# Samleo8/RadarSLAMPy

Hardware: AMD Instinct MI355X
Metric: radar scan-pairs/sec (400x3768 polar) (higher is better)
Workload: dtype u8/f32/f64

## Files before the change

radarslampy_amd/csrc/engine.hip:

```cpp
#include "roam_internal.h"
#include "retrack.h"
#include "kabsch_body.inc"
#include <algorithm>
#include <new>

#define KS ROAM_MAX_FEATURES
#define CART_CENTER 1012.0
#define M_PER_PX 0.0864
#define N_RETRACK 60
#define ROT_THR 0.2
#define TRANS_THR_SQ 4.0
#define ERR_THR 10.0f
#define TWO_PI 6.283185307179586476925286766559

#define RES_RING 8
enum { ST_PEAKS = 0, ST_WARP, ST_PYR, ST_KLT, ST_GRAPH, ST_CLIQUE, ST_KABSCH, ST_LM, ST_GLUE, ST_RETRACK, ST_COUNT };
static const char *kStageNames[ST_COUNT] = {"ingest_peaks", "warp_quantise", "pyramid", "klt", "consistency_graph",
                                            "max_clique", "kabsch", "mds_lm", "glue", "retrack"};

struct Engine {
    roam_engine_cfg cfg;
    int B = 0, W = 0, stage_cap = 0;
    PyrDesc pd;
    size_t rec_bytes = 0;
// ... 39 lines not shown
    hipEvent_t ev_pool = nullptr;
    bool pool_dirty = false;
    RtArgs rt;
    bool rt_on = false;
    int rt_mode = 1;
    uint8_t *kfb = nullptr;
    uint8_t *rmap = nullptr;
    int rmap_cap = 0;
    int64_t rmap_n = 0;
    int64_t rmap_n_bcast = 0;
    std::vector<int32_t> rmap_root;
    uint8_t *kfx_send = nullptr, *kfx_recv = nullptr;
    size_t kfx_rec = 0;
    int kfx_peaks = 0;
    int kfx_world = 0;
    int64_t *rmap_n_dev = nullptr;
    int32_t *rmap_root_dev = nullptr;
    int64_t kfx_calls = 0;
    bool kfx_ready = false;
    hipStream_t st_comm = nullptr;
    hipEvent_t ev_kfx[3] = {};
    int kfx_last = -1;
    hipEvent_t ev[ST_COUNT + 1] = {};
    bool stage_ev_forced = false;
    bool stage_ev = true;
    hipEvent_t ev_join = nullptr, ev_pk0 = nullptr, ev_pk1 = nullptr;
    hipEvent_t ev_klt[4] = {}, ev_g4[4] = {};
    hipEvent_t ev_warp = nullptr;
    hipEvent_t ev_idx = nullptr, ev_peaks = nullptr;
    hipEvent_t tr_ev[64][6] = {};
    hipEvent_t rt_ev[64][3 * RT_TRACE_CHUNKS] = {};
    bool rt_ev_ok[64] = {};
    hipEvent_t ev_emit = nullptr;
    RtSide det_side = {};
    int det_chunk() const { return (det_side.chunk > 0 && retrack_sided(rt, B, &det_side)) ? det_side.chunk : rt.slots; }
    int64_t rt_image_px = 0;
    bool tr_ev_ok[64] = {};
    int64_t stage_ev_step = -1;
    bool tr_ok = false;
    unsigned long long *pyr_dark = nullptr;
    static constexpr bool warp_dark_zero = true;
    bool ev_ok = false, stepped = false, uploads_pending = false;
    uint64_t up_seq = 0, up_waited = 0;
    std::vector<uint64_t> slot_seq;
    hipEvent_t ev_up_ring[16] = {};
    std::vector<int> lane_k;
// ... 76 lines not shown
            good_new[2 * o] = klt_next[2 * i]; good_new[2 * o + 1] = klt_next[2 * i + 1];
            good_idx[o] = k;
            pos++;
        }
    }
    if (t == 0) good_n[b] = total;
}

__global__ void fill_mask_kernel(uint8_t *mask, const int32_t *good_n, int32_t *cq_n, int32_t *cq_flags)
{
    const int b = blockIdx.x;
    for (int k = threadIdx.x; k < KS; k += blockDim.x) mask[(int64_t)b * KS + k] = 1;
    if (threadIdx.x == 0) { cq_n[b] = good_n[b]; cq_flags[b] = 1; }
}

__global__ __launch_bounds__(256) void g2_inliers_kernel(const float *__restrict__ good_old, const float *__restrict__ good_new,
                                                         const int32_t *__restrict__ good_idx, const int32_t *__restrict__ good_n,
                                                         const uint8_t *__restrict__ mask, const double *__restrict__ kf_pose,
                                                         const double *__restrict__ kf_und, double *__restrict__ kf_und_tmp,
                                                         double *__restrict__ kab_src, double *__restrict__ kab_tgt,
                                                         double *__restrict__ p_w, double *__restrict__ p_jt,
                                                         float *__restrict__ feat, int32_t *__restrict__ in_n,
                                                         double *__restrict__ kab_out, const double *__restrict__ pose,
                                                         double *__restrict__ T_wj0, double *__restrict__ T_init)
{
    __shared__ int sh[8];
    __shared__ double red[8];
    const int b = blockIdx.x, t = threadIdx.x;
    const int G = good_n[b];
    const int items = (KS + 255) / 256;
    const int lo = t * items, hi = min(lo + items, G);
    int c = 0;
    for (int g = lo; g < hi; g++) c += mask[(int64_t)b * KS + g] ? 1 : 0;
    int total;
    int pos = blk_excl_scan(c, sh, &total);
    const double kx = kf_pose[3 * b], ky = kf_pose[3 * b + 1], kth = kf_pose[3 * b + 2];
    const double ck = cos(kth), sk = sin(kth);
    for (int g = lo; g < hi; g++) {
        const int64_t i = (int64_t)b * KS + g;
        if (!mask[i]) continue;
        const int64_t o = (int64_t)b * KS + pos;
        const float ox = good_old[2 * i], oy = good_old[2 * i + 1];
        const float nx = good_new[2 * i], ny = good_new[2 * i + 1];
        kab_src[2 * o] = (double)ox; kab_src[2 * o + 1] = (double)oy;
        kab_tgt[2 * o] = (double)nx; kab_tgt[2 * o + 1] = (double)ny;
        const int64_t ki = (int64_t)b * KS + good_idx[i];
        const double ux = kf_und[2 * ki], uy = kf_und[2 * ki + 1];
        kf_und_tmp[2 * o] = ux; kf_und_tmp[2 * o + 1] = uy;
        p_w[2 * o] = ck * ux - sk * uy + kx;
        p_w[2 * o + 1] = sk * ux + ck * uy + ky;
        p_jt[2 * o] = ((double)nx - CART_CENTER) * M_PER_PX;
        p_jt[2 * o + 1] = ((double)ny - CART_CENTER) * M_PER_PX;
        pos++;
    }
    __syncthreads();
    pos -= c;
    for (int g = lo; g < hi; g++) {
        const int64_t i = (int64_t)b * KS + g;
        if (!mask[i]) continue;
        const int64_t o = (int64_t)b * KS + pos;
        feat[2 * o] = good_new[2 * i]; feat[2 * o + 1] = good_new[2 * i + 1];
        pos++;
    }
    if (t == 0) in_n[b] = total;
    __threadfence_block();
    __syncthreads();
    double *ko = kab_out + 6 * (int64_t)b;
    kabsch_body(kab_src + (int64_t)b * KS * 2, kab_tgt + (int64_t)b * KS * 2, total, red, ko);
    if (T_wj0 && t == 0) {
        const double x = pose[3 * b], y = pose[3 * b + 1], th = pose[3 * b + 2];
        const double c = cos(th), s = sin(th);
        double *T0 = T_wj0 + 9 * (int64_t)b, *Ti = T_init + 9 * (int64_t)b;
        T0[0] = c; T0[1] = -s; T0[2] = x; T0[3] = s; T0[4] = c; T0[5] = y; T0[6] = 0; T0[7] = 0; T0[8] = 1;
        const double hx = ko[4] * M_PER_PX, hy = ko[5] * M_PER_PX;
        Ti[0] = c * ko[0] - s * ko[2]; Ti[1] = c * ko[1] - s * ko[3]; Ti[2] = c * hx - s * hy + x;
        Ti[3] = s * ko[0] + c * ko[2]; Ti[4] = s * ko[1] + c * ko[3]; Ti[5] = s * hx + c * hy + y;
        Ti[6] = 0; Ti[7] = 0; Ti[8] = 1;
    }
}


#define MAP_SLOT (8 + 2 * KS)
__device__ __forceinline__ void map_freeze(double *__restrict__ map_store, int32_t *__restrict__ map_n, int map_cap, int b,
                                           const double *__restrict__ kfp, const double *__restrict__ kfv, int n,
                                           int scan, const double *__restrict__ locals)
{
    const int slot = map_n[b];
    if (slot >= map_cap) return;
    double *d = map_store + ((size_t)b * map_cap + slot) * MAP_SLOT;
    for (int j = threadIdx.x; j < 2 * n; j += blockDim.x) d[8 + j] = locals[j];
    if (threadIdx.x == 0) {
        d[0] = kfp[0]; d[1] = kfp[1]; d[2] = kfp[2];
        d[3] = kfv[0]; d[4] = kfv[1]; d[5] = kfv[2];
        d[6] = (double)n; d[7] = (double)scan;
    }
}

__global__ __launch_bounds__(256) void map_freeze_kernel(double *__restrict__ map_store, int32_t *__restrict__ map_n, int map_cap,
                                                         int b, const double *__restrict__ kf_pose,
                                                         const double *__restrict__ kf_vel, const int32_t *__restrict__ feat_n,
                                                         const int32_t *__restrict__ kf_scan, const double *__restrict__ kf_und,
                                                         const int32_t *__restrict__ kf_live, const int32_t *__restrict__ kf_fresh)
{
    if (!kf_live[b] || kf_fresh[b]) return;
    const int slot = map_n[b];
    map_freeze(map_store, map_n, map_cap, b, kf_pose + 3 * b, kf_vel + 3 * b, feat_n[b], kf_scan[b], kf_und + (size_t)b * KS * 2);
    __syncthreads();
    if (threadIdx.x == 0 && slot < map_cap) map_n[b] = slot + 1;
}

__global__ __launch_bounds__(256) void g4_update_kernel(roam_engine_cfg cfg, const double *__restrict__ lm_out,
                                                        const int32_t *__restrict__ lm_nfev, const int32_t *__restrict__ lm_info,
                                                        const double *__restrict__ kab_out, double *__restrict__ pose,
                                                        double *__restrict__ vel, double *__restrict__ kf_pose,
                                                        double *__restrict__ kf_und, const double *__restrict__ kf_und_tmp,
                                                        const double *__restrict__ p_jt, const int32_t *__restrict__ in_n,
                                                        const int32_t *__restrict__ good_n, int32_t *__restrict__ feat_n,
                                                        const int32_t *__restrict__ peaks_n, const int32_t *__restrict__ cq_flags,
                                                        roam_lane_result *__restrict__ res, const int32_t *__restrict__ scan_idx,
                                                        double *__restrict__ kf_vel, int32_t *__restrict__ kf_scan,
                                                        int32_t *__restrict__ kf_fresh, const int32_t *__restrict__ kf_live,
                                                        double *__restrict__ map_store, int32_t *__restrict__ map_n, int map_cap,
                                                        int collect, int32_t *__restrict__ rt_lane, int32_t *__restrict__ rt_scan,
                                                        int32_t *__restrict__ rt_n)
{
    __shared__ double np_[3], nv_[3];
    __shared__ int newkf;
    const int b = blockIdx.x, t = threadIdx.x;
    const int n = in_n[b];
    if (t == 0) {
        double px = pose[3 * b], py = pose[3 * b + 1], pth = pose[3 * b + 2];
        double v0 = 0, v1 = 0, v2 = 0;
        const double *k = kab_out + 6 * (int64_t)b;
        if (n >= 2) {
            if (cfg.motion_distortion) {
                const double *s = lm_out + 6 * (int64_t)b;
                v0 = s[0]; v1 = s[1]; v2 = s[2]; px = s[3]; py = s[4]; pth = s[5];
            } else {
                const double dx = k[4] * M_PER_PX, dy = k[5] * M_PER_PX, dth = atan2(k[2], k[0]);
                const double c = cos(pth), s = sin(pth);
                px += dx * c - dy * s; py += dx * s + dy * c; pth += dth;
            }
        }
        np_[0] = px; np_[1] = py; np_[2] = pth; nv_[0] = v0; nv_[1] = v1; nv_[2] = v2;
        const int retrack = n <= N_RETRACK;
        const double dth = fabs(kf_pose[3 * b + 2] - pth);
        const double ddx = kf_pose[3 * b] - px, ddy = kf_pose[3 * b + 1] - py;
        const int good = (dth >= cfg.keyframe_rot_rad) || (ddx * ddx + ddy * ddy >= cfg.keyframe_trans_m * cfg.keyframe_trans_m);
        newkf = retrack || good;
        roam_lane_result *r = res + b;
        r->pose[0] = px; r->pose[1] = py; r->pose[2] = pth;
        r->velocity[0] = v0; r->velocity[1] = v1; r->velocity[2] = v2;
        r->kabsch_R[0] = k[0]; r->kabsch_R[1] = k[1]; r->kabsch_R[2] = k[2]; r->kabsch_R[3] = k[3];
        r->kabsch_h[0] = k[4] * M_PER_PX; r->kabsch_h[1] = k[5] * M_PER_PX;
        r->n_tracked = feat_n[b]; r->n_good = good_n[b]; r->n_inliers = n; r->n_peaks = peaks_n[b];
        r->lm_nfev = (n >= 2 && cfg.motion_distortion) ? lm_nfev[b] : 0;
        r->lm_info = (n >= 2 && cfg.motion_distortion) ? lm_info[b] : 0;
        __hip_atomic_store(&r->flags, (cq_flags[b] & 1) | (newkf ? 2 : 0) | (retrack ? 4 : 0), __ATOMIC_RELAXED, __HIP_MEMORY_SCOPE_AGENT);
        r->n_after_retrack = 0;
    }
    __syncthreads();
    const double v0 = nv_[0], v1 = nv_[1], v2 = nv_[2];
    const int mslot = (newkf && map_cap > 0 && kf_live[b]) ? map_n[b] : -1;
    if (mslot >= 0) map_freeze(map_store, map_n, map_cap, b, kf_pose + 3 * b, kf_vel + 3 * b, n, kf_scan[b], kf_und_tmp + (int64_t)b * KS * 2);
    for (int j = t; j < n; j += 256) {
        const int64_t o = (int64_t)b * KS + j;
        if (newkf) {
            const double x = p_jt[2 * o], y = p_jt[2 * o + 1];
            const double dT = 0.25 * atan2(-y, -x) / TWO_PI;
            const double a = v2 * dT, ca = cos(a), sa = sin(a);
            kf_und[2 * o] = ca * x - sa * y + v0 * dT;
            kf_und[2 * o + 1] = sa * x + ca * y + v1 * dT;
        } else {
            kf_und[2 * o] = kf_und_tmp[2 * o]; kf_und[2 * o + 1] = kf_und_tmp[2 * o + 1];
        }
    }
    __syncthreads();
    if (t == 0) {
        pose[3 * b] = np_[0]; pose[3 * b + 1] = np_[1]; pose[3 * b + 2] = np_[2];
        vel[3 * b] = v0; vel[3 * b + 1] = v1; vel[3 * b + 2] = v2;
        if (newkf) {
            kf_pose[3 * b] = np_[0]; kf_pose[3 * b + 1] = np_[1]; kf_pose[3 * b + 2] = np_[2];
            kf_vel[3 * b] = v0; kf_vel[3 * b + 1] = v1; kf_vel[3 * b + 2] = v2;
            kf_scan[b] = scan_idx[b];
            if (mslot >= 0 && mslot < map_cap) map_n[b] = mslot + 1;
        }
        kf_fresh[b] = newkf;
        feat_n[b] = n;
    }
    if (collect) {
        __shared__ int last_s, sh[4], base_s;
#if defined(__HIP_DEVICE_COMPILE__) && !defined(__gfx942__) && !defined(__gfx950__)
#error "g4_update_kernel's hand-off to its last block relies on gfx94x/95x storing with write-through and counting stores in vmcnt: s_waitcnt vmcnt(0) + relaxed atomics, no release/acquire pair"
#endif
        asm volatile("s_waitcnt vmcnt(0)" ::: "memory");
        __syncthreads();
        if (t == 0) last_s = atomicAdd(rt_n + 1, 1) == (int)gridDim.x - 1;
        __syncthreads();
        if (!last_s) return;
        const int B = (int)gridDim.x;
        if (t == 0) base_s = 0;
        __syncthreads();
        for (int b0 = 0; b0 < B; b0 += 256) {
            const int bb = b0 + t;
            const int f = (bb < B && (collect == 2 || (__hip_atomic_load(&res[bb].flags, __ATOMIC_RELAXED, __HIP_MEMORY_SCOPE_AGENT) & 4))) ? 1 : 0;
            const int lane = t & 63, w = t >> 6;
            int inc = f;
#pragma unroll
            for (int d = 1; d < 64; d <<= 1) { const int nn = __shfl_up(inc, d); if (lane >= d) inc += nn; }
            if (lane == 63) sh[w] = inc;
            __syncthreads();
            int off = base_s, tot = 0;
            for (int i = 0; i < 4; i++) { if (i < w) off += sh[i]; tot += sh[i]; }
            if (f) { rt_lane[off + inc - 1] = bb; rt_scan[off + inc - 1] = scan_idx[bb]; }
            __syncthreads();
            if (t == 0) base_s += tot;
            __syncthreads();
        }
        if (t == 0) { rt_n[0] = base_s; rt_n[1] = 0; }
    }
}

__global__ void lane_kf_reset_kernel(const float *__restrict__ feat, int K, const double *__restrict__ vel,
                                     double *__restrict__ kf_und)
{
    const int j = blockIdx.x * blockDim.x + threadIdx.x;
    if (j >= K) return;
    const double x = ((double)feat[2 * j] - CART_CENTER) * M_PER_PX, y = ((double)feat[2 * j + 1] - CART_CENTER) * M_PER_PX;
    const double dT = 0.25 * atan2(-y, -x) / TWO_PI;
    const double a = vel[2] * dT, ca = cos(a), sa = sin(a);
    kf_und[2 * j] = ca * x - sa * y + vel[0] * dT;
    kf_und[2 * j + 1] = sa * x + ca * y + vel[1] * dT;
}

#define KFB_HDR 64
#define KFB_LOCALS_OFF KFB_HDR
#define KFB_PEAKS_OFF (KFB_HDR + KS * 16)
__global__ __launch_bounds__(256) void kf_pack_kernel(uint8_t *__restrict__ buf, int lane, const double *__restrict__ kf_pose,
                                                      const double *__restrict__ kf_vel, const int32_t *__restrict__ feat_n,
                                                      const int32_t *__restrict__ kf_scan, const double *__restrict__ kf_und,
                                                      const int32_t *__restrict__ peaks_n, const int32_t *__restrict__ peaks,
                                                      int peaks_cap)
// ... 73 lines not shown
{
    const int rec = blockIdx.y, row = blockIdx.x * 4 + (threadIdx.x >> 6), lane = threadIdx.x & 63;
    if (row >= rows) return;
    const uint8_t *s = host + (int64_t)rec * host_stride + (int64_t)row * stride;
    uint8_t *d = pool + (int64_t)rec * rec_bytes + (int64_t)row * stride;
    const int nvec = width / 16;
    for (int v = lane; v < nvec; v += 64) *reinterpret_cast<u32x4_a1 *>(d + 16 * v) = *reinterpret_cast<const u32x4_a1 *>(s + 16 * v);
    for (int b = nvec * 16 + lane; b < width; b += 64) d[b] = s[b];
}

extern "C" {

int32_t roam_engine_destroy(roam_ctx *ctx)
{
    if (!ctx) return ROAM_E_ARG;
    Engine *e = ctx->engine;
    if (!e) return ROAM_OK;
    hipSetDevice(ctx->device);
    hipStreamSynchronize(ctx->stream);
    for (void *p : e->allocs) hipFree(p);
    auto kill = [](hipEvent_t &ev) { if (ev) { hipEventDestroy(ev); ev = nullptr; } };
    for (auto &ev : e->ev) kill(ev);
    for (int i = 0; i < 4; i++) { kill(e->det_side.ev_i[i]); kill(e->det_side.ev_d[i]); }
    kill(e->ev_emit);
    kill(e->ev_join); kill(e->ev_pk0); kill(e->ev_pk1); kill(e->ev_warp); kill(e->ev_idx); kill(e->ev_peaks);
    for (int i = 0; i < 4; i++) { kill(e->ev_klt[i]); kill(e->ev_g4[i]); }
    for (auto &row : e->tr_ev) for (auto &ev : row) kill(ev);
    for (auto &row : e->rt_ev) for (auto &ev : row) kill(ev);
    if (e->scan_host) hipHostFree(e->scan_host);
    if (e->results_host) hipHostFree(e->results_host);
    for (auto &ev : e->ev_res) if (ev) hipEventDestroy(ev);
    if (e->st_comm) { hipStreamSynchronize(e->st_comm); hipStreamDestroy(e->st_comm); }
    for (auto &ev : e->ev_kfx) if (ev) hipEventDestroy(ev);
    if (e->ev_pool) hipEventDestroy(e->ev_pool);
    for (auto &ev : e->ev_up_ring) if (ev) hipEventDestroy(ev);
    hipStreamSynchronize(ctx->stream2);
    hipStreamSynchronize(ctx->stream4);
    delete e;
    ctx->engine = nullptr;
    return ROAM_OK;
}

static int32_t fused_tables(roam_ctx *ctx, Engine *e)
{
    RtArgs &r = e->rt;
    if (r.fd_mapT) return ROAM_OK;
    const size_t npx = (size_t)e->W * e->W, R = (size_t)r.slots;
// ... 124 lines not shown
        ok = ok && dalloc(ctx, e, &r.ssc_work, D * 4 * BP_MAX_PTS) && dalloc(ctx, e, &r.sel, D * BP_MAX_PTS) && dalloc(ctx, e, &r.sel_n, D) && dalloc(ctx, e, &r.blob_order_buf, D);
    }
    if (!ok) { roam_engine_destroy(ctx); return ROAM_E_HIP; }
    if (e->rt_on) {
        if (hipError_t er = retrack_init(); er != hipSuccess) {
            ROAM_SET_ERR(ctx, "retrack_init failed: %s", hipGetErrorString(er));
            roam_engine_destroy(ctx);
            return ROAM_E_HIP;
        }
        RtArgs &r = e->rt;
        r.pool = e->pool; r.map = e->warp_map; r.feat = e->feat; r.feat_n = e->feat_n; r.vel = e->vel; r.kf_und = e->kf_und; r.res = nullptr;
    }
    for (auto &ev : e->ev_res)
        if (hipEventCreateWithFlags(&ev, hipEventDisableTiming) != hipSuccess) { ROAM_SET_ERR(ctx, "hipEventCreate failed"); roam_engine_destroy(ctx); return ROAM_E_HIP; }
    e->slot_seq.assign((size_t)cfg->pool_scans, 0);
    for (auto &ev : e->ev_up_ring)
        if (hipEventCreateWithFlags(&ev, hipEventDisableTiming) != hipSuccess) { ROAM_SET_ERR(ctx, "hipEventCreate failed"); roam_engine_destroy(ctx); return ROAM_E_HIP; }
    if (hipEventCreateWithFlags(&e->ev_pool, hipEventDisableTiming) != hipSuccess) {
        ROAM_SET_ERR(ctx, "hipEventCreate failed"); roam_engine_destroy(ctx); return ROAM_E_HIP;
    }
    for (auto &ev : e->ev) {
        if (hipEventCreate(&ev) != hipSuccess) { ROAM_SET_ERR(ctx, "hipEventCreate failed"); roam_engine_destroy(ctx); return ROAM_E_HIP; }
    }
    if (hipEventCreate(&e->ev_join) != hipSuccess ||
        hipEventCreate(&e->ev_pk0) != hipSuccess || hipEventCreate(&e->ev_pk1) != hipSuccess ||
        hipEventCreateWithFlags(&e->ev_warp, hipEventDisableTiming) != hipSuccess || hipEventCreateWithFlags(&e->ev_idx, hipEventDisableTiming) != hipSuccess ||
        hipEventCreateWithFlags(&e->ev_peaks, hipEventDisableTiming) != hipSuccess) {
        ROAM_SET_ERR(ctx, "hipEventCreate failed"); roam_engine_destroy(ctx); return ROAM_E_HIP;
    }
    for (int i = 0; i < 4; i++)
        if (hipEventCreateWithFlags(&e->ev_klt[i], hipEventDisableTiming) != hipSuccess || hipEventCreateWithFlags(&e->ev_g4[i], hipEventDisableTiming) != hipSuccess) {
            ROAM_SET_ERR(ctx, "hipEventCreate failed"); roam_engine_destroy(ctx); return ROAM_E_HIP;
        }
    e->ev_ok = true;
    e->tr_ok = true;
    HIP_TRY(ctx, launch_warp_map(ctx->stream, cfg->rows, cfg->clip, e->warp_map));
    HIP_TRY(ctx, launch_pyr_dark(ctx->stream, e->warp_map, e->W, e->W, cfg->clip, e->pyr_dark));
    if (e->rt_on) HIP_TRY(ctx, launch_retrack_boxtab(ctx->stream, e->warp_map, e->W, cfg->clip, const_cast<uint32_t *>(e->rt.boxtab)));
    if (e->rt_on) HIP_TRY(ctx, launch_retrack_darktab(ctx->stream, e->warp_map, e->W, cfg->clip, const_cast<uint32_t *>(e->rt.darktab)));
    if (e->rt_on && e->rt.fused) { const int32_t rc_ = fused_tables(ctx, e); if (rc_ != ROAM_OK) { roam_engine_destroy(ctx); return rc_; } }
    HIP_TRY(ctx, hipStreamSynchronize(ctx->stream));
    e->rt_image_px = (int64_t)e->W * e->W;
    if (e->rt_on && e->W <= 2048 && B >= RT_TWO_PASS_SLOTS) {
        e->rt_image_px = 0;
        const size_t npx = (size_t)e->W * e->W, ndt = retrack_darktab_words(e->W), nph = retrack_phase_words(e->W);
        uint32_t *stage = nullptr;
        HIP_TRY(ctx, hipHostMalloc(reinterpret_cast<void **>(&stage), (npx + ndt + nph) * 4, hipHostMallocDefault));
// ... 511 lines not shown
    HIP_TRY(ctx, hipEventRecord(e->ev_join, sB));
    HIP_TRY(ctx, hipStreamWaitEvent(st, e->ev_join, 0));
    if (e->stage_ev) HIP_TRY(ctx, hipEventRecord(e->ev[ST_KLT], st));
    if (any_new) {
        hipLaunchKernelGGL(new_sequence_kernel, dim3((B + 255) / 256), dim3(256), 0, st, e->feat_n, e->scan_idx[pb] + B, B);
        HIP_TRY(ctx, hipGetLastError());
    }
    HIP_TRY(ctx, launch_klt(st, prev, next, e->pd, e->feat, e->feat_n, KM, KS, B, e->klt_next, e->klt_status, e->klt_err));
    HIP_TRY(ctx, hipEventRecord(e->ev_klt[k4], st));
    hipLaunchKernelGGL(g1_good_kernel, dim3(B), dim3(256), 0, st, e->feat, e->feat_n, e->klt_next, e->klt_status, e->klt_err,
                       e->good_old, e->good_new, e->good_idx, e->good_n, KM);
    HIP_TRY(ctx, hipGetLastError());
    if (e->stage_ev) HIP_TRY(ctx, hipEventRecord(e->ev[ST_GRAPH], st));
    if (c.reject_outliers) {
        HIP_TRY(ctx, launch_consistency_graph(st, e->good_old, e->good_new, e->good_n, KM, KS, B, 0.5 / M_PER_PX, e->adj, nw));
        if (e->stage_ev) HIP_TRY(ctx, hipEventRecord(e->ev[ST_CLIQUE], st));
        HIP_TRY(ctx, launch_max_clique(st, e->adj, e->good_n, KM, KS, nw, B, c.clique_node_limit, e->cq_stack, e->cq_mask, e->cq_n, e->cq_flags, e->cq_order));
    } else {
        if (e->stage_ev) HIP_TRY(ctx, hipEventRecord(e->ev[ST_CLIQUE], st));
        hipLaunchKernelGGL(fill_mask_kernel, dim3(B), dim3(256), 0, st, e->cq_mask, e->good_n, e->cq_n, e->cq_flags);
        HIP_TRY(ctx, hipGetLastError());
    }
    if (e->stage_ev) HIP_TRY(ctx, hipEventRecord(e->ev[ST_KABSCH], st));
    hipLaunchKernelGGL(g2_inliers_kernel, dim3(B), dim3(256), 0, st, e->good_old, e->good_new, e->good_idx, e->good_n, e->cq_mask,
                       e->kf_pose, e->kf_und, e->kf_und_tmp, e->kab_src, e->kab_tgt, e->p_w, e->p_jt, e->feat, e->in_n, e->kab_out, e->pose,
                       c.motion_distortion ? e->T_wj0 : nullptr, e->T_init);
    HIP_TRY(ctx, hipGetLastError());
    if (e->stage_ev) HIP_TRY(ctx, hipEventRecord(e->ev[ST_LM], st));
    if (c.motion_distortion) {
        MdsProblemDesc P;
        P.T_wj0 = e->T_wj0; P.T_init = e->T_init; P.p_w = e->p_w; P.p_jt = e->p_jt; P.count = e->in_n;
        P.N = KM; P.nstride = KS; P.nmax = KM; P.B = B; P.period = 0.25;
        for (int i = 0; i < 5; i++) P.sigma5[i] = c.sigma5[i];
        P.big = e->lm_big; P.big_slot = e->lm_big_slot; e->lm_big_slot ^= 1;
        HIP_TRY(ctx, launch_mds_solve(st, P, e->lm_work, e->lm_out, e->lm_nfev, e->lm_info, nullptr, nullptr));
    }
    if (e->stage_ev) HIP_TRY(ctx, hipEventRecord(e->ev[ST_GLUE], st));
    HIP_TRY(ctx, hipStreamWaitEvent(st, e->ev_peaks, 0));
    hipLaunchKernelGGL(g4_update_kernel, dim3(B), dim3(256), 0, st, c, e->lm_out, e->lm_nfev, e->lm_info, e->kab_out, e->pose,
                       e->vel, e->kf_pose, e->kf_und, e->kf_und_tmp, e->p_jt, e->in_n, e->good_n, e->feat_n, e->peaks_n[pb],
                       e->cq_flags, res_slot, e->scan_idx[pb], e->kf_vel, e->kf_scan, e->kf_fresh, e->kf_live, e->map_store, e->map_n,
                       e->map_cap, (e->rt_on && e->rt_mode) ? (e->rt_mode == 2 ? 2 : 1) : 0, e->rt.rt_lane, e->rt.rt_scan, e->rt.rt_n);
    HIP_TRY(ctx, hipGetLastError());
    if (e->stage_ev) HIP_TRY(ctx, hipEventRecord(e->ev[ST_RETRACK], st));
    if (e->rt_on && e->rt_mode) {
        e->rt.res = res_slot;
        if (B >= 256 && !e->ev_emit) HIP_TRY(ctx, hipEventCreateWithFlags(&e->ev_emit, hipEventDisableTiming));
        if (e->det_side.chunk > 0 && !e->det_side.ev_i[0]) {
            e->det_side.st = sB;
            for (int i = 0; i < 4; i++) { HIP_TRY(ctx, hipEventCreateWithFlags(&e->det_side.ev_i[i], hipEventDisableTiming)); HIP_TRY(ctx, hipEventCreateWithFlags(&e->det_side.ev_d[i], hipEventDisableTiming)); }
        }
        HIP_TRY(ctx, launch_retrack(st, e->rt, B, e->stage_ev ? e->rt_ev[e->nstep & 63] : nullptr, RT_TRACE_CHUNKS, e->ev_emit,
                                    e->det_side.chunk > 0 ? &e->det_side : nullptr));
        if (e->rt_mode == 2) e->rt_floor = std::min(KS, e->kmax() + 256);
    }
    e->rt_ev_ok[e->nstep & 63] = e->rt_on && e->rt_mode && e->stage_ev;
    if (e->stage_ev) HIP_TRY(ctx, hipEventRecord(e->ev[ST_COUNT], st));
    HIP_TRY(ctx, hipEventRecord(e->ev_g4[k4], st));
    HIP_TRY(ctx, hipMemcpyAsync(e->results_host + (size_t)rs * B, res_slot, sizeof(roam_lane_result) * (size_t)B, hipMemcpyDeviceToHost, st));
    HIP_TRY(ctx, hipEventRecord(e->ev_res[rs], st));
    e->cur = (e->cur + 1) & 3;
    e->pk = pb;
    e->nstep++;
    e->stepped = true;
    return ROAM_OK;
}

int32_t roam_engine_results(roam_ctx *ctx, roam_lane_result *out, int32_t n)
{
    ENGINE();
    ARG_CHECK(ctx, out && n >= 1 && n <= e->B);
    if (e->nstep == 0) { ROAM_SET_ERR(ctx, "no step enqueued"); return ROAM_E_STATE; }
    return roam_engine_step_results(ctx, e->nstep - 1, out, n);
}

int32_t roam_engine_step_results(roam_ctx *ctx, int64_t step, roam_lane_result *out, int32_t n)
{
    ENGINE();
// ... 106 lines not shown
}

int32_t roam_engine_set_stage_events(roam_ctx *ctx, int32_t on)
{
    ENGINE();
    if (!e->stage_ev_forced) e->stage_ev = on != 0;
    return ROAM_OK;
}

int32_t roam_engine_stage_times(roam_ctx *ctx, float *ms_out, const char **names_out, int32_t cap, int32_t *n)
{
    ENGINE();
    ARG_CHECK(ctx, ms_out && n && cap >= ST_COUNT);
    if (!e->stepped) { ROAM_SET_ERR(ctx, "no step recorded"); return ROAM_E_STATE; }
    if (!e->stage_ev) { ROAM_SET_ERR(ctx, "stage events are off (roam_engine_set_stage_events)"); return ROAM_E_STATE; }
    if (e->stage_ev_step != e->nstep - 1) { ROAM_SET_ERR(ctx, "the last step was enqueued with stage events off: run a step first"); return ROAM_E_STATE; }
    HIP_TRY(ctx, hipStreamSynchronize(ctx->stream));
    for (int i = 0; i < ST_COUNT; i++) {
        float ms = 0;
        hipEvent_t *tl = e->tr_ev[(e->nstep - 1) & 63];
        if (i == ST_PEAKS) HIP_TRY(ctx, hipEventElapsedTime(&ms, tl[0], tl[5]));
        else if (i == ST_WARP) HIP_TRY(ctx, hipEventElapsedTime(&ms, tl[1], tl[2]));
        else if (i == ST_PYR) HIP_TRY(ctx, hipEventElapsedTime(&ms, tl[3], tl[4]));
        else HIP_TRY(ctx, hipEventElapsedTime(&ms, e->ev[i], e->ev[i + 1]));
        ms_out[i] = ms;
        if (names_out) names_out[i] = kStageNames[i];
    }
    *n = ST_COUNT;
    return ROAM_OK;
}

int32_t roam_engine_kernel_avg(roam_ctx *ctx, const char *name, int32_t last_steps, float *avg_ms, int32_t *n_used)
{
    ENGINE();
    ARG_CHECK(ctx, name && last_steps >= 1 && avg_ms && n_used);
    if (!e->stage_ev) { ROAM_SET_ERR(ctx, "stage events are off (roam_engine_set_stage_events)"); return ROAM_E_STATE; }
    int k = !strcmp(name, "ingest_peaks") ? 0 : (!strcmp(name, "warp_quantise") ? 1 : (!strcmp(name, "pyramid") ? 2 : -1));
    const int kd = !strcmp(name, "doh_integral") ? 0 : (!strcmp(name, "doh_det_maxima") ? 1 : -1);
    if (k < 0 && kd < 0) { ROAM_SET_ERR(ctx, "unknown kernel '%s'", name); return ROAM_E_ARG; }
    if (kd >= 0 && !e->rt_on) { ROAM_SET_ERR(ctx, "engine created without retrack_on_device"); return ROAM_E_STATE; }
    if (!e->stepped) { ROAM_SET_ERR(ctx, "run a step first"); return ROAM_E_STATE; }
    HIP_TRY(ctx, hipStreamSynchronize(ctx->stream));
    int64_t n = std::min<int64_t>(std::min<int64_t>(last_steps, e->nstep), 64);
    double sum = 0;
    if (kd >= 0) {
        int64_t used = 0;
// ... 154 lines not shown
```

radarslampy_amd/csrc/retrack.h:

```cpp
#pragma once
#include "roam_internal.h"
#include "blobprune.h"

#define RT_TWO_PASS_SLOTS 200
enum { RT_F_CAND_OVERFLOW = 1, RT_F_TREE_OVERFLOW = 2, RT_F_PAIR_OVERFLOW = 4, RT_F_FEAT_OVERFLOW = 8 };

struct RtArgs {
    int W, rows, cols, stride, payload_off, slots, size1, size2;
    int64_t rec_bytes;
    double sigma1, sigma2, threshold;
    const uint8_t *pool;
    const uint32_t *map;
    const uint32_t *phlist;
    const uint32_t *boxtab;
    const uint32_t *darktab;
    float *feat;
    int32_t *feat_n;
    const double *vel;
    double *kf_und;
    roam_lane_result *res;
    int32_t *rt_n, *rt_lane, *rt_scan;
    double *S;
    int32_t *col_done;
    double *colT;
// ... 6 lines not shown
    uint16_t *order;
    uint32_t *ovbits;
    uint16_t *bigtab;
    double *kp;
    int32_t *kp_n, *slot_flags;
    int32_t *ssc_work;
    int32_t *sel, *sel_n;
    int32_t *blob_order_buf;
    const int32_t *blob_order;
    int fused;
    const uint32_t *fd_mapT;
    const uint32_t *fd_boxtab;
    const uint32_t *fd_darktab;
    double *fd_halo;
    int64_t fd_halo_words;
    double *fd_cc;
};

hipError_t launch_retrack_collect(hipStream_t st, const roam_lane_result *res, const int32_t *scan_idx, int B, int force_all, const RtArgs &a);
#define RT_TRACE_CHUNKS 16
struct RtSide { hipStream_t st; hipEvent_t ev_i[4], ev_d[4]; int chunk; };
bool retrack_sided(const RtArgs &a, int B, const RtSide *side);
hipError_t launch_retrack(hipStream_t st, const RtArgs &a, int B, hipEvent_t *trace = nullptr, int ntrace = 0, hipEvent_t after_order = nullptr, const RtSide *side = nullptr);
hipError_t launch_ssc_batch(hipStream_t st, const double *kp, int64_t kp_stride, const int32_t *count, int kp_cap, int P,
                            int num_ret, double tol, int cols, int rows, int32_t *work, int32_t *sel, int32_t *n_sel,
                            const int32_t *n_active, int first);
hipError_t launch_retrack_part(hipStream_t st, const RtArgs &a, int P, int which);
hipError_t launch_retrack_emit(hipStream_t st, const RtArgs &a, int P);
hipError_t retrack_init();
size_t retrack_boxtab_words(int W);
size_t retrack_phase_words(int W);
int retrack_band_rows();
bool retrack_build_phases(const uint32_t *map_host, const uint32_t *darktab_host, int W, int cols, uint32_t *out);
hipError_t launch_retrack_boxtab(hipStream_t st, const uint32_t *map, int W, int cols, uint32_t *boxtab);
size_t retrack_darktab_words(int W);
size_t retrack_fused_boxtab_words(int W);
size_t retrack_fused_halo_words(int W);
hipError_t launch_retrack_fused_tables(hipStream_t st, const uint32_t *map, int W, int cols, uint32_t *mapT, uint32_t *boxtab, uint32_t *darktab);
hipError_t launch_retrack_darktab(hipStream_t st, const uint32_t *map, int W, int cols, uint32_t *darktab);
```

radarslampy_amd/csrc/retrack.hip:

```cpp
#include "retrack_geom.h"

#define KS ROAM_MAX_FEATURES
#define CART_CENTER 1012.0
#define M_PER_PX 0.0864
#define TWO_PI 6.283185307179586476925286766559

__global__ __launch_bounds__(256) void rt_collect_kernel(const roam_lane_result *__restrict__ res, const int32_t *__restrict__ scan_idx,
                                                         int B, int force_all, int32_t *__restrict__ rt_lane,
                                                         int32_t *__restrict__ rt_scan, int32_t *__restrict__ rt_n)
{
    __shared__ int sh[8];
    __shared__ int base_s;
    const int t = threadIdx.x;
    if (t == 0) base_s = 0;
    __syncthreads();
    for (int b0 = 0; b0 < B; b0 += 256) {
        const int b = b0 + t;
        const int f = (b < B && (force_all || (res[b].flags & 4))) ? 1 : 0;
        const int lane = t & 63, w = t >> 6;
        int inc = f;
#pragma unroll
        for (int d = 1; d < 64; d <<= 1) { int n = __shfl_up(inc, d); if (lane >= d) inc += n; }
        if (lane == 63) sh[w] = inc;
        __syncthreads();
// ... 50 lines not shown
            if (pos < KS) {
                feat[2 * pos] = nx[i]; feat[2 * pos + 1] = ny[i];
                const double x = ((double)nx[i] - CART_CENTER) * M_PER_PX, y = ((double)ny[i] - CART_CENTER) * M_PER_PX;
                const double dT = 0.25 * atan2(-y, -x) / TWO_PI;
                const double ang = v2 * dT, ca = cos(ang), sa = sin(ang);
                und[2 * pos] = ca * x - sa * y + v0 * dT;
                und[2 * pos + 1] = sa * x + ca * y + v1 * dT;
            }
            pos++;
        }
    if (t == 0) {
        a.feat_n[b] = m;
        if (a.res) {
            a.res[b].flags |= 8 | (a.slot_flags[ls] << 8) | ((total > KS || a.sel_n[ls] > 256) ? (RT_F_FEAT_OVERFLOW << 8) : 0);
            a.res[b].n_after_retrack = m;
        }
    }
}

hipError_t retrack_init() { const hipError_t e = retrack_det_init(); return e != hipSuccess ? e : retrack_integral_init(); }

bool retrack_sided(const RtArgs &a, int B, const RtSide *side) { return side && side->chunk > 0 && !a.fused && a.slots >= 2 * side->chunk && B > side->chunk; }

hipError_t launch_retrack(hipStream_t st, const RtArgs &a, int B, hipEvent_t *trace, int ntrace, hipEvent_t after_order, const RtSide *side)
{
    if (a.W > 2048) return hipErrorInvalidValue;
    const bool sided = retrack_sided(a, B, side);
    const int C = sided ? side->chunk : a.slots;
    const hipStream_t dst = sided ? side->st : st;
    hipError_t e = hipSuccess;
    int nc = 0;
    for (int first = 0; first < B; first += C, nc++) {
        const int P = min(C, B - first);
        const bool tr = trace && nc < ntrace, big = B - first >= RT_TWO_PASS_SLOTS;
        hipEvent_t *tev = trace + 3 * nc;
        RtArgs ac = a;
        if (sided) ac.S = a.S + (size_t)(nc & 1) * C * a.SP * a.W;
        if (sided && nc >= 2 && (e = hipStreamWaitEvent(st, side->ev_d[(nc - 2) & 3], 0)) != hipSuccess) return e;
        if (tr && (e = hipEventRecord(tev[0], st)) != hipSuccess) return e;
        if (big && a.fused && (e = launch_retrack_fused(st, ac, first, P, 0)) != hipSuccess) return e;
        if ((e = launch_retrack_integral(st, ac, first, P, big && !a.fused)) != hipSuccess) return e;
        if (tr && (e = hipEventRecord(tev[1], st)) != hipSuccess) return e;
        if (sided && (e = hipEventRecord(side->ev_i[nc & 3], st)) != hipSuccess) return e;
        if (sided && (e = hipStreamWaitEvent(dst, side->ev_i[nc & 3], 0)) != hipSuccess) return e;
        if ((e = launch_det(dst, ac, first, P)) != hipSuccess) return e;
        if (tr && (e = hipEventRecord(tev[2], dst)) != hipSuccess) return e;
        if (sided && (e = hipEventRecord(side->ev_d[nc & 3], dst)) != hipSuccess) return e;
    }
    for (int k = max(0, nc - 2); sided && k < nc; k++)
        if ((e = hipStreamWaitEvent(st, side->ev_d[k & 3], 0)) != hipSuccess) return e;
    if ((e = launch_retrack_bookkeeping(st, a, B, after_order)) != hipSuccess) return e;
    hipLaunchKernelGGL(rt_append_kernel, dim3(B), dim3(256), 0, st, a, 0);
    return hipGetLastError();
}

hipError_t launch_retrack_collect(hipStream_t st, const roam_lane_result *res, const int32_t *scan_idx, int B, int force_all, const RtArgs &a)
{
    hipLaunchKernelGGL(rt_collect_kernel, dim3(1), dim3(256), 0, st, res, scan_idx, B, force_all, a.rt_lane, a.rt_scan, a.rt_n);
    return hipGetLastError();
}

hipError_t launch_retrack_part(hipStream_t st, const RtArgs &a_in, int P, int which)
{
    if (a_in.W > 2048) return hipErrorInvalidValue;
    RtArgs a = a_in;
    a.fused = which >= 2 ? 1 : 0;
    if (which >= 2) return a.fd_mapT ? launch_retrack_fused(st, a, 0, P, which - 2) : hipErrorInvalidValue;
    if (which == 0) return launch_retrack_integral(st, a, 0, P, true);
    return launch_det(st, a, 0, P);
}
```

Baseline: 53670.

## Build retrack lane list in inliers kernel and overlap retrack with LM solve

Moves the last-block retrack lane-list collection from the g4 update kernel into g2_inliers_kernel, keyed on inlier count instead of the result flags. Because the retrack list is known earlier, the MDS LM solve and g4 update can run on a side stream while the retrack image and detection passes run on the main stream, joining before bookkeeping and append. The aim is to hide the LM solve latency behind the retrack work. The risks are contention on the side stream, which the detection chunks also use, and the new criterion (in_n <= N_RETRACK) possibly not matching the old retrack flag exactly.

```diff
diff --git a/radarslampy_amd/csrc/engine.hip b/radarslampy_amd/csrc/engine.hip
--- a/radarslampy_amd/csrc/engine.hip
+++ b/radarslampy_amd/csrc/engine.hip
@@ -85,6 +85,8 @@
     hipEvent_t ev_kfx[3] = {};
     int kfx_last = -1;
     hipEvent_t ev[ST_COUNT + 1] = {};
+    hipEvent_t ev_glue_end = nullptr;
+    hipEvent_t ev_list = nullptr, ev_lm = nullptr;
     bool stage_ev_forced = false;
     bool stage_ev = true;
     hipEvent_t ev_join = nullptr, ev_pk0 = nullptr, ev_pk1 = nullptr;
@@ -207,7 +209,9 @@
                                                          double *__restrict__ p_w, double *__restrict__ p_jt,
                                                          float *__restrict__ feat, int32_t *__restrict__ in_n,
                                                          double *__restrict__ kab_out, const double *__restrict__ pose,
-                                                         double *__restrict__ T_wj0, double *__restrict__ T_init)
+                                                         double *__restrict__ T_wj0, double *__restrict__ T_init, int collect,
+                                                         const int32_t *__restrict__ scan_idx, int32_t *__restrict__ rt_lane,
+                                                         int32_t *__restrict__ rt_scan, int32_t *__restrict__ rt_n)
 {
     __shared__ int sh[8];
     __shared__ double red[8];
@@ -247,7 +251,7 @@
         feat[2 * o] = good_new[2 * i]; feat[2 * o + 1] = good_new[2 * i + 1];
         pos++;
     }
-    if (t == 0) in_n[b] = total;
+    if (t == 0) __hip_atomic_store(in_n + b, total, __ATOMIC_RELAXED, __HIP_MEMORY_SCOPE_AGENT);
     __threadfence_block();
     __syncthreads();
     double *ko = kab_out + 6 * (int64_t)b;
@@ -262,6 +266,37 @@
         Ti[3] = s * ko[0] + c * ko[2]; Ti[4] = s * ko[1] + c * ko[3]; Ti[5] = s * hx + c * hy + y;
         Ti[6] = 0; Ti[7] = 0; Ti[8] = 1;
     }
+    if (collect) {
+        __shared__ int last_s, cs[4], base_s;
+#if defined(__HIP_DEVICE_COMPILE__) && !defined(__gfx942__) && !defined(__gfx950__)
+#error "g2_inliers_kernel's hand-off to its last block relies on gfx94x/95x storing with write-through and counting stores in vmcnt: s_waitcnt vmcnt(0) + relaxed atomics, no release/acquire pair"
+#endif
+        asm volatile("s_waitcnt vmcnt(0)" ::: "memory");
+        __syncthreads();
+        if (t == 0) last_s = atomicAdd(rt_n + 1, 1) == (int)gridDim.x - 1;
+        __syncthreads();
+        if (!last_s) return;
+        const int B = (int)gridDim.x;
+        if (t == 0) base_s = 0;
+        __syncthreads();
+        for (int b0 = 0; b0 < B; b0 += 256) {
+            const int bb = b0 + t;
+            const int f = (bb < B && (collect == 2 || __hip_atomic_load(in_n + bb, __ATOMIC_RELAXED, __HIP_MEMORY_SCOPE_AGENT) <= N_RETRACK)) ? 1 : 0;
+            const int lane = t & 63, w = t >> 6;
+            int inc = f;
+#pragma unroll
+            for (int d = 1; d < 64; d <<= 1) { const int nn = __shfl_up(inc, d); if (lane >= d) inc += nn; }
+            if (lane == 63) cs[w] = inc;
+            __syncthreads();
+            int off = base_s, tot = 0;
+            for (int i = 0; i < 4; i++) { if (i < w) off += cs[i]; tot += cs[i]; }
+            if (f) { rt_lane[off + inc - 1] = bb; rt_scan[off + inc - 1] = scan_idx[bb]; }
+            __syncthreads();
+            if (t == 0) base_s += tot;
+            __syncthreads();
+        }
+        if (t == 0) { rt_n[0] = base_s; rt_n[1] = 0; }
+    }
 }
 
 
@@ -305,9 +340,7 @@
                                                         roam_lane_result *__restrict__ res, const int32_t *__restrict__ scan_idx,
                                                         double *__restrict__ kf_vel, int32_t *__restrict__ kf_scan,
                                                         int32_t *__restrict__ kf_fresh, const int32_t *__restrict__ kf_live,
-                                                        double *__restrict__ map_store, int32_t *__restrict__ map_n, int map_cap,
-                                                        int collect, int32_t *__restrict__ rt_lane, int32_t *__restrict__ rt_scan,
-                                                        int32_t *__restrict__ rt_n)
+                                                        double *__restrict__ map_store, int32_t *__restrict__ map_n, int map_cap)
 {
     __shared__ double np_[3], nv_[3];
     __shared__ int newkf;
@@ -341,7 +374,7 @@
         r->n_tracked = feat_n[b]; r->n_good = good_n[b]; r->n_inliers = n; r->n_peaks = peaks_n[b];
         r->lm_nfev = (n >= 2 && cfg.motion_distortion) ? lm_nfev[b] : 0;
         r->lm_info = (n >= 2 && cfg.motion_distortion) ? lm_info[b] : 0;
-        __hip_atomic_store(&r->flags, (cq_flags[b] & 1) | (newkf ? 2 : 0) | (retrack ? 4 : 0), __ATOMIC_RELAXED, __HIP_MEMORY_SCOPE_AGENT);
+        r->flags = (cq_flags[b] & 1) | (newkf ? 2 : 0) | (retrack ? 4 : 0);
         r->n_after_retrack = 0;
     }
     __syncthreads();
@@ -372,37 +405,6 @@
         }
         kf_fresh[b] = newkf;
         feat_n[b] = n;
-    }
-    if (collect) {
-        __shared__ int last_s, sh[4], base_s;
-#if defined(__HIP_DEVICE_COMPILE__) && !defined(__gfx942__) && !defined(__gfx950__)
-#error "g4_update_kernel's hand-off to its last block relies on gfx94x/95x storing with write-through and counting stores in vmcnt: s_waitcnt vmcnt(0) + relaxed atomics, no release/acquire pair"
-#endif
-        asm volatile("s_waitcnt vmcnt(0)" ::: "memory");
-        __syncthreads();
-        if (t == 0) last_s = atomicAdd(rt_n + 1, 1) == (int)gridDim.x - 1;
-        __syncthreads();
-        if (!last_s) return;
-        const int B = (int)gridDim.x;
-        if (t == 0) base_s = 0;
-        __syncthreads();
-        for (int b0 = 0; b0 < B; b0 += 256) {
-            const int bb = b0 + t;
-            const int f = (bb < B && (collect == 2 || (__hip_atomic_load(&res[bb].flags, __ATOMIC_RELAXED, __HIP_MEMORY_SCOPE_AGENT) & 4))) ? 1 : 0;
-            const int lane = t & 63, w = t >> 6;
-            int inc = f;
-#pragma unroll
-            for (int d = 1; d < 64; d <<= 1) { const int nn = __shfl_up(inc, d); if (lane >= d) inc += nn; }
-            if (lane == 63) sh[w] = inc;
-            __syncthreads();
-            int off = base_s, tot = 0;
-            for (int i = 0; i < 4; i++) { if (i < w) off += sh[i]; tot += sh[i]; }
-            if (f) { rt_lane[off + inc - 1] = bb; rt_scan[off + inc - 1] = scan_idx[bb]; }
-            __syncthreads();
-            if (t == 0) base_s += tot;
-            __syncthreads();
-        }
-        if (t == 0) { rt_n[0] = base_s; rt_n[1] = 0; }
     }
 }
 
@@ -522,7 +524,7 @@
     auto kill = [](hipEvent_t &ev) { if (ev) { hipEventDestroy(ev); ev = nullptr; } };
     for (auto &ev : e->ev) kill(ev);
     for (int i = 0; i < 4; i++) { kill(e->det_side.ev_i[i]); kill(e->det_side.ev_d[i]); }
-    kill(e->ev_emit);
+    kill(e->ev_emit); kill(e->ev_glue_end); kill(e->ev_list); kill(e->ev_lm);
     kill(e->ev_join); kill(e->ev_pk0); kill(e->ev_pk1); kill(e->ev_warp); kill(e->ev_idx); kill(e->ev_peaks);
     for (int i = 0; i < 4; i++) { kill(e->ev_klt[i]); kill(e->ev_g4[i]); }
     for (auto &row : e->tr_ev) for (auto &ev : row) kill(ev);
@@ -693,7 +695,7 @@
     for (auto &ev : e->ev) {
         if (hipEventCreate(&ev) != hipSuccess) { ROAM_SET_ERR(ctx, "hipEventCreate failed"); roam_engine_destroy(ctx); return ROAM_E_HIP; }
     }
-    if (hipEventCreate(&e->ev_join) != hipSuccess ||
+    if (hipEventCreate(&e->ev_join) != hipSuccess || hipEventCreate(&e->ev_glue_end) != hipSuccess ||
         hipEventCreate(&e->ev_pk0) != hipSuccess || hipEventCreate(&e->ev_pk1) != hipSuccess ||
         hipEventCreateWithFlags(&e->ev_warp, hipEventDisableTiming) != hipSuccess || hipEventCreateWithFlags(&e->ev_idx, hipEventDisableTiming) != hipSuccess ||
         hipEventCreateWithFlags(&e->ev_peaks, hipEventDisableTiming) != hipSuccess) {
@@ -1251,38 +1253,57 @@
         HIP_TRY(ctx, hipGetLastError());
     }
     if (e->stage_ev) HIP_TRY(ctx, hipEventRecord(e->ev[ST_KABSCH], st));
+    const bool detect = e->rt_on && e->rt_mode;
     hipLaunchKernelGGL(g2_inliers_kernel, dim3(B), dim3(256), 0, st, e->good_old, e->good_new, e->good_idx, e->good_n, e->cq_mask,
                        e->kf_pose, e->kf_und, e->kf_und_tmp, e->kab_src, e->kab_tgt, e->p_w, e->p_jt, e->feat, e->in_n, e->kab_out, e->pose,
-                       c.motion_distortion ? e->T_wj0 : nullptr, e->T_init);
+                       c.motion_distortion ? e->T_wj0 : nullptr, e->T_init,
+                       detect ? (e->rt_mode == 2 ? 2 : 1) : 0, e->scan_idx[pb], e->rt.rt_lane, e->rt.rt_scan, e->rt.rt_n);
     HIP_TRY(ctx, hipGetLastError());
-    if (e->stage_ev) HIP_TRY(ctx, hipEventRecord(e->ev[ST_LM], st));
+    if (detect) {
+        e->rt.res = res_slot;
+        if (B >= 256 && !e->ev_emit) HIP_TRY(ctx, hipEventCreateWithFlags(&e->ev_emit, hipEventDisableTiming));
+        if (e->det_side.chunk > 0 && !e->det_side.ev_i[0]) {
+            e->det_side.st = sB;
+            for (int i = 0; i < 4; i++) { HIP_TRY(ctx, hipEventCreateWithFlags(&e->det_side.ev_i[i], hipEventDisableTiming)); HIP_TRY(ctx, hipEventCreateWithFlags(&e->det_side.ev_d[i], hipEventDisableTiming)); }
+        }
+    }
+    hipEvent_t *rtr = e->stage_ev ? e->rt_ev[e->nstep & 63] : nullptr;
+    const RtSide *side = e->det_side.chunk > 0 ? &e->det_side : nullptr;
+    const bool early = detect && c.motion_distortion && B >= 256;
+    hipStream_t sL = early ? sB : st;
+    if (early) {
+        if (!e->ev_list) { HIP_TRY(ctx, hipEventCreateWithFlags(&e->ev_list, hipEventDisableTiming)); HIP_TRY(ctx, hipEventCreateWithFlags(&e->ev_lm, hipEventDisableTiming)); }
+        HIP_TRY(ctx, hipEventRecord(e->ev_list, st));
+        HIP_TRY(ctx, hipStreamWaitEvent(sL, e->ev_list, 0));
+    }
+    if (e->stage_ev) HIP_TRY(ctx, hipEventRecord(e->ev[ST_LM], sL));
     if (c.motion_distortion) {
         MdsProblemDesc P;
         P.T_wj0 = e->T_wj0; P.T_init = e->T_init; P.p_w = e->p_w; P.p_jt = e->p_jt; P.count = e->in_n;
         P.N = KM; P.nstride = KS; P.nmax = KM; P.B = B; P.period = 0.25;
         for (int i = 0; i < 5; i++) P.sigma5[i] = c.sigma5[i];
         P.big = e->lm_big; P.big_slot = e->lm_big_slot; e->lm_big_slot ^= 1;
-        HIP_TRY(ctx, launch_mds_solve(st, P, e->lm_work, e->lm_out, e->lm_nfev, e->lm_info, nullptr, nullptr));
-    }
-    if (e->stage_ev) HIP_TRY(ctx, hipEventRecord(e->ev[ST_GLUE], st));
-    HIP_TRY(ctx, hipStreamWaitEvent(st, e->ev_peaks, 0));
-    hipLaunchKernelGGL(g4_update_kernel, dim3(B), dim3(256), 0, st, c, e->lm_out, e->lm_nfev, e->lm_info, e->kab_out, e->pose,
+        HIP_TRY(ctx, launch_mds_solve(sL, P, e->lm_work, e->lm_out, e->lm_nfev, e->lm_info, nullptr, nullptr));
+    }
+    if (e->stage_ev) HIP_TRY(ctx, hipEventRecord(e->ev[ST_GLUE], sL));
+    HIP_TRY(ctx, hipStreamWaitEvent(sL, e->ev_peaks, 0));
+    hipLaunchKernelGGL(g4_update_kernel, dim3(B), dim3(256), 0, sL, c, e->lm_out, e->lm_nfev, e->lm_info, e->kab_out, e->pose,
                        e->vel, e->kf_pose, e->kf_und, e->kf_und_tmp, e->p_jt, e->in_n, e->good_n, e->feat_n, e->peaks_n[pb],
                        e->cq_flags, res_slot, e->scan_idx[pb], e->kf_vel, e->kf_scan, e->kf_fresh, e->kf_live, e->map_store, e->map_n,
-                       e->map_cap, (e->rt_on && e->rt_mode) ? (e->rt_mode == 2 ? 2 : 1) : 0, e->rt.rt_lane, e->rt.rt_scan, e->rt.rt_n);
+                       e->map_cap);
     HIP_TRY(ctx, hipGetLastError());
-    if (e->stage_ev) HIP_TRY(ctx, hipEventRecord(e->ev[ST_RETRACK], st));
-    if (e->rt_on && e->rt_mode) {
-        e->rt.res = res_slot;
-        if (B >= 256 && !e->ev_emit) HIP_TRY(ctx, hipEventCreateWithFlags(&e->ev_emit, hipEventDisableTiming));
-        if (e->det_side.chunk > 0 && !e->det_side.ev_i[0]) {
-            e->det_side.st = sB;
-            for (int i = 0; i < 4; i++) { HIP_TRY(ctx, hipEventCreateWithFlags(&e->det_side.ev_i[i], hipEventDisableTiming)); HIP_TRY(ctx, hipEventCreateWithFlags(&e->det_side.ev_d[i], hipEventDisableTiming)); }
-        }
-        HIP_TRY(ctx, launch_retrack(st, e->rt, B, e->stage_ev ? e->rt_ev[e->nstep & 63] : nullptr, RT_TRACE_CHUNKS, e->ev_emit,
-                                    e->det_side.chunk > 0 ? &e->det_side : nullptr));
-        if (e->rt_mode == 2) e->rt_floor = std::min(KS, e->kmax() + 256);
-    }
+    if (e->stage_ev) HIP_TRY(ctx, hipEventRecord(e->ev_glue_end, sL));
+    if (early) {
+        HIP_TRY(ctx, hipEventRecord(e->ev_lm, sL));
+        if (e->stage_ev) HIP_TRY(ctx, hipEventRecord(e->ev[ST_RETRACK], st));
+        HIP_TRY(ctx, launch_retrack_images(st, e->rt, B, rtr, RT_TRACE_CHUNKS, side));
+        HIP_TRY(ctx, hipStreamWaitEvent(st, e->ev_lm, 0));
+        HIP_TRY(ctx, launch_retrack_finish(st, e->rt, B, e->ev_emit, side));
+    } else {
+        if (e->stage_ev) HIP_TRY(ctx, hipEventRecord(e->ev[ST_RETRACK], st));
+        if (detect) HIP_TRY(ctx, launch_retrack(st, e->rt, B, rtr, RT_TRACE_CHUNKS, e->ev_emit, side));
+    }
+    if (detect && e->rt_mode == 2) e->rt_floor = std::min(KS, e->kmax() + 256);
     e->rt_ev_ok[e->nstep & 63] = e->rt_on && e->rt_mode && e->stage_ev;
     if (e->stage_ev) HIP_TRY(ctx, hipEventRecord(e->ev[ST_COUNT], st));
     HIP_TRY(ctx, hipEventRecord(e->ev_g4[k4], st));
@@ -1435,6 +1456,7 @@
         if (i == ST_PEAKS) HIP_TRY(ctx, hipEventElapsedTime(&ms, tl[0], tl[5]));
         else if (i == ST_WARP) HIP_TRY(ctx, hipEventElapsedTime(&ms, tl[1], tl[2]));
         else if (i == ST_PYR) HIP_TRY(ctx, hipEventElapsedTime(&ms, tl[3], tl[4]));
+        else if (i == ST_GLUE) HIP_TRY(ctx, hipEventElapsedTime(&ms, e->ev[ST_GLUE], e->ev_glue_end));
         else HIP_TRY(ctx, hipEventElapsedTime(&ms, e->ev[i], e->ev[i + 1]));
         ms_out[i] = ms;
         if (names_out) names_out[i] = kStageNames[i];
diff --git a/radarslampy_amd/csrc/retrack.h b/radarslampy_amd/csrc/retrack.h
--- a/radarslampy_amd/csrc/retrack.h
+++ b/radarslampy_amd/csrc/retrack.h
@@ -52,6 +52,8 @@
 struct RtSide { hipStream_t st; hipEvent_t ev_i[4], ev_d[4]; int chunk; };
 bool retrack_sided(const RtArgs &a, int B, const RtSide *side);
 hipError_t launch_retrack(hipStream_t st, const RtArgs &a, int B, hipEvent_t *trace = nullptr, int ntrace = 0, hipEvent_t after_order = nullptr, const RtSide *side = nullptr);
+hipError_t launch_retrack_images(hipStream_t st, const RtArgs &a, int B, hipEvent_t *trace, int ntrace, const RtSide *side);
+hipError_t launch_retrack_finish(hipStream_t st, const RtArgs &a, int B, hipEvent_t after_order, const RtSide *side);
 hipError_t launch_ssc_batch(hipStream_t st, const double *kp, int64_t kp_stride, const int32_t *count, int kp_cap, int P,
                             int num_ret, double tol, int cols, int rows, int32_t *work, int32_t *sel, int32_t *n_sel,
                             const int32_t *n_active, int first);
diff --git a/radarslampy_amd/csrc/retrack.hip b/radarslampy_amd/csrc/retrack.hip
--- a/radarslampy_amd/csrc/retrack.hip
+++ b/radarslampy_amd/csrc/retrack.hip
@@ -96,7 +96,7 @@
 
 bool retrack_sided(const RtArgs &a, int B, const RtSide *side) { return side && side->chunk > 0 && !a.fused && a.slots >= 2 * side->chunk && B > side->chunk; }
 
-hipError_t launch_retrack(hipStream_t st, const RtArgs &a, int B, hipEvent_t *trace, int ntrace, hipEvent_t after_order, const RtSide *side)
+hipError_t launch_retrack_images(hipStream_t st, const RtArgs &a, int B, hipEvent_t *trace, int ntrace, const RtSide *side)
 {
     if (a.W > 2048) return hipErrorInvalidValue;
     const bool sided = retrack_sided(a, B, side);
@@ -121,11 +121,25 @@
         if (tr && (e = hipEventRecord(tev[2], dst)) != hipSuccess) return e;
         if (sided && (e = hipEventRecord(side->ev_d[nc & 3], dst)) != hipSuccess) return e;
     }
+    return e;
+}
+
+hipError_t launch_retrack_finish(hipStream_t st, const RtArgs &a, int B, hipEvent_t after_order, const RtSide *side)
+{
+    const bool sided = retrack_sided(a, B, side);
+    const int C = sided ? side->chunk : a.slots, nc = (B + C - 1) / C;
+    hipError_t e = hipSuccess;
     for (int k = max(0, nc - 2); sided && k < nc; k++)
         if ((e = hipStreamWaitEvent(st, side->ev_d[k & 3], 0)) != hipSuccess) return e;
     if ((e = launch_retrack_bookkeeping(st, a, B, after_order)) != hipSuccess) return e;
     hipLaunchKernelGGL(rt_append_kernel, dim3(B), dim3(256), 0, st, a, 0);
     return hipGetLastError();
+}
+
+hipError_t launch_retrack(hipStream_t st, const RtArgs &a, int B, hipEvent_t *trace, int ntrace, hipEvent_t after_order, const RtSide *side)
+{
+    const hipError_t e = launch_retrack_images(st, a, B, trace, ntrace, side);
+    return e != hipSuccess ? e : launch_retrack_finish(st, a, B, after_order, side);
 }
 
 hipError_t launch_retrack_collect(hipStream_t st, const roam_lane_result *res, const int32_t *scan_idx, int B, int force_all, const RtArgs &a)
```

Measured after the change: 52210. -2.7%, worse.
